# dataexplorations2026/cough_detector

Measured on AMD Instinct MI355X. Metric: 1s@16kHz clips/sec (featurise+infer), higher is better.
Workload: dtype bf16x3: split-bf16 MFMA (feature image, activations and BN-folded weights as hi+lo bf16 pairs, 3 v_mfma_f32_32x32x16_bf16 per k-step, f32 accumulate, f32 activations in HBM); featuriser f32

## Files before the change

### cough_detector_amd/csrc/common.h

```cpp
#pragma once
#include <hip/hip_runtime.h>

#include <cstdarg>
#include <cstdio>

#include "../../include/cough_amd.h"

namespace cough {

void set_error(const char* fmt, ...);

#define COUGH_DEFINE_LAST_ERROR(entry_point)                                  \
    namespace cough {                                                         \
    namespace {                                                               \
    thread_local char g_last_error[512] = "";                                 \
    }                                                                         \
    void set_error(const char* fmt, ...) {                                    \
        va_list ap;                                                           \
        va_start(ap, fmt);                                                    \
        vsnprintf(g_last_error, sizeof(g_last_error), fmt, ap);               \
        va_end(ap);                                                           \
    }                                                                         \
    }                                                                         \
    extern "C" const char* entry_point(void) { return cough::g_last_error; }

inline bool aligned(const void* p, size_t a) { return (reinterpret_cast<size_t>(p) & (a - 1)) == 0; }

#define COUGH_HIP_CHECK(expr)                                                              \
    do {                                                                                   \
        hipError_t _e = (expr);                                                            \
        if (_e != hipSuccess) {                                                            \
            ::cough::set_error("%s failed: %s (%s:%d)", #expr, hipGetErrorString(_e), __FILE__, __LINE__); \
            return COUGH_EHIP;                                                             \
        }                                                                                  \
    } while (0)

#define COUGH_REQUIRE(cond, code, ...)       \
    do {                                     \
        if (!(cond)) {                       \
            ::cough::set_error(__VA_ARGS__); \
            return (code);                   \
        }                                    \
    } while (0)

template <int CTRL, int ROW_MASK = 0xf>
__device__ __forceinline__ float dpp_mov(float v) {
    return __int_as_float(__builtin_amdgcn_update_dpp(0, __float_as_int(v), CTRL, ROW_MASK, 0xf, false));
}
__device__ __forceinline__ float wave_max(float v) {
    v = fmaxf(v, dpp_mov<0xB1>(v));
    v = fmaxf(v, dpp_mov<0x4E>(v));
    v = fmaxf(v, dpp_mov<0x141>(v));
    v = fmaxf(v, dpp_mov<0x140>(v));
    v = fmaxf(v, __shfl_xor(v, 16, 64));
    v = fmaxf(v, __shfl_xor(v, 32, 64));
    return v;
}
__device__ __forceinline__ float wave_sum(float v) {
    v += dpp_mov<0xB1>(v);
    v += dpp_mov<0x4E>(v);
    v += dpp_mov<0x141>(v);
    v += dpp_mov<0x140>(v);
    v += __shfl_xor(v, 16, 64);
    v += __shfl_xor(v, 32, 64);
    return v;
}

__device__ __forceinline__ float mul_rn(float a, float b) {
    float r;
    asm volatile("v_mul_f32 %0, %1, %2" : "=v"(r) : "v"(a), "v"(b));
    return r;
}

__device__ __forceinline__ void wave_lds_fence() {
    __builtin_amdgcn_fence(__ATOMIC_ACQ_REL, "wavefront");
    __builtin_amdgcn_wave_barrier();
}

}
```

### cough_detector_amd/csrc/featurize.hip

```cpp
#include <cmath>
#include <cstddef>
#include <cstring>
#include <type_traits>
#include <vector>

#include <hip/hip_bf16.h>

#include <cstdlib>

#include "common.h"
#include "fft256.h"
#include "internal.h"

namespace cough {
namespace {

constexpr int NS = 16000, NFFT = 512, HOP = 160, WIN = 400, NFRAMES = 101, NMEL = 64, NMFCC = 13;
constexpr int PADL = NFFT / 2;
constexpr int NBIN = 128;
constexpr int MAXW = 8;
constexpr int THREADS = 256, WAVES = THREADS / 64;
constexpr int FPW = 4;
constexpr int NGROUP = (NFRAMES + FPW - 1) / FPW;
constexpr int XROW = 17;
constexpr int XFRAME = 16 * XROW;
constexpr int NMF = NMFCC * NFRAMES;
constexpr int FIRST_PLAIN = 2, LAST_PLAIN = 98;

struct FeatTables {
    float win[NFFT];
    float2 tw256[16][16];
    float2 tw512[NBIN];
    int mel_start[NMEL];
    float mel_w[NMEL][MAXW];
    float dct_t[NMFCC + 1][NMEL];
};

constexpr size_t LDS_XCH = size_t(WAVES) * FPW * XFRAME * 4;
constexpr size_t LDS_MEL = size_t(NMEL) * NFRAMES * 4;
constexpr size_t LDS_RED = 16 * 4;
constexpr size_t LDS_TW = size_t(16) * XROW * 8;
constexpr size_t LDS_TOTAL = LDS_XCH + LDS_MEL + LDS_RED + LDS_TW;
static_assert(LDS_TOTAL * 3 <= 160 * 1024, "three workgroups per CU");
static_assert(LDS_XCH >= size_t(2) * NMF * 4, "MFCC / delta buffers alias the transpose scratch");

__device__ __forceinline__ float block_max(float v, float* red, int tid) {
    v = wave_max(v);
    __syncthreads();
    if ((tid & 63) == 0) red[tid >> 6] = v;
    __syncthreads();
    float r = red[0];
#pragma unroll
    for (int w = 1; w < WAVES; ++w) r = fmaxf(r, red[w]);
    return r;
}
__device__ __forceinline__ float block_sum(float v, float* red, int tid) {
    v = wave_sum(v);
    __syncthreads();
    if ((tid & 63) == 0) red[tid >> 6] = v;
    __syncthreads();
    float r = red[0];
#pragma unroll
    for (int w = 1; w < WAVES; ++w) r += red[w];
    return r;
}

#ifdef COUGH_K1_STAMPS
__device__ unsigned long long* g_stamp_buf = nullptr;
#define K1_STAMP(slot)                                                                      \
    do {                                                                                    \
        if (g_stamp_buf && threadIdx.x == 0)                                                \
            g_stamp_buf[(size_t)blockIdx.x * 8 + (slot)] = __builtin_amdgcn_s_memtime();    \
    } while (0)
#else
#define K1_STAMP(slot) do { } while (0)
#endif

#ifdef COUGH_K1_MARKERS
#define K1_MARK(text)                             \
    do {                                          \
        __builtin_amdgcn_sched_barrier(0);        \
        asm volatile("; K1MARK " text);           \
        __builtin_amdgcn_sched_barrier(0);        \
    } while (0)
#else
#define K1_MARK(text) do { } while (0)
#endif

using f32x16 = __attribute__((ext_vector_type(16))) float;
using bf16x8 = __attribute__((ext_vector_type(8))) __bf16;
__device__ __forceinline__ uint16_t f2bf(float f) {
    __hip_bfloat16 b = __float2bfloat16(f);
    return *reinterpret_cast<uint16_t*>(&b);
}
constexpr int ST_P1H = 22, ST_P1W = 25, ST_ROWS = 94;
constexpr int ST_PER = ST_P1H * ST_P1W, ST_TILES = (ST_PER + 7) / 8;
constexpr int ST_PITCH_NARROW = 106, ST_PITCH_WIDE = 112;
constexpr int st_pitch(bool full) { return full ? ST_PITCH_NARROW : ST_PITCH_WIDE; }
constexpr size_t st_img(bool full) { return size_t(ST_ROWS) * st_pitch(full) * 2; }
static_assert((2 * (ST_PITCH_WIDE / 2)) % 32 == 16 && ST_PITCH_WIDE % 2 == 0, "wide pitch: dy moves a fragment 16 banks on");
static_assert(st_img(false) <= LDS_MEL, "the bf16 feature image aliases the dB buffer");
constexpr size_t LDS_WG3_MAX = 53760;
constexpr size_t st_x3_off(bool full) { return full ? LDS_TOTAL - 2 * st_img(true) : (size_t(NMF) * 4 + 15) & ~size_t(15); }
constexpr size_t LDS_X3_WIDE = st_x3_off(false) + 2 * st_img(false);
static_assert(st_x3_off(false) % 16 == 0 && st_x3_off(true) % 16 == 0 && st_img(false) % 4 == 0 && st_img(true) % 4 == 0 &&
              st_x3_off(true) >= size_t(NMF) * 4, "hi / lo images vs the MFCC buffer");
static_assert(LDS_X3_WIDE >= LDS_TOTAL && LDS_X3_WIDE <= LDS_WG3_MAX, "the widened split-bf16 stem keeps three workgroups per CU");
constexpr size_t shipped_lds_bytes(int stem) { return stem == 2 ? LDS_X3_WIDE : LDS_TOTAL; }

struct FullBank {
    int n_mels, n_mfcc, n_taps;
    int maxw[2];
    int n_frames, n_samples, hop;
    int cph, cph_pad, cw;
    const int *lo, *hi, *off;
    const float* w;
    const float* dct;
};
constexpr size_t full_mel_bytes(int n_mels, int n_frames = NFRAMES) { return (size_t(n_mels) * n_frames * 4 + 15) & ~size_t(15); }
constexpr int FX_ROW = FPW * 16 + 1, FX_WAVE = 16 * FX_ROW, FX_PROW = 260;
static_assert(FPW * FX_PROW <= FX_WAVE && FX_PROW >= NFFT / 2 + 2 && FX_PROW % 2 == 0, "four power rows replace the transposes");
constexpr size_t LDS_XCH_FULL = size_t(WAVES) * FX_WAVE * 4;
constexpr int FULL_MAX_MFCC = int(LDS_XCH_FULL / (size_t(2) * NFRAMES * 4));
constexpr size_t full_lds_bytes(int n_mels, int n_taps, int n_frames = NFRAMES) {
    return LDS_XCH_FULL + full_mel_bytes(n_mels, n_frames) + LDS_RED + LDS_TW + ((size_t(n_taps) * 4 + 15) & ~size_t(15));
}

#ifndef COUGH_GEO_WG_PER_CU
#define COUGH_GEO_WG_PER_CU 2
#endif
template <bool PRE_EMPH, int STEM, bool FULL = false, bool TALL = false, bool PCS = false, bool GEO = false>
__global__ __launch_bounds__(THREADS, GEO ? COUGH_GEO_WG_PER_CU : 3) void featurize_kernel(
    const float* __restrict__ wav, long long wav_stride, float* __restrict__ out, int nfeat,
    const FeatTables* __restrict__ tb, int normalize, float pre_coef, int delta_delta , int pcen, StemFuse stem, FullBank fbk,
    const float* __restrict__ full_dct ,
    float* __restrict__ peak_out ) {
    extern __shared__ __attribute__((aligned(16))) char smem[];
    static_assert(!GEO || (FULL && STEM == 0 && !TALL && !PCS), "run-time geometry: full-band instantiations without a stem");
    constexpr int ST_PITCH = st_pitch(FULL);
    constexpr size_t ST_X3_OFF = st_x3_off(FULL);
    static_assert(FULL || shipped_lds_bytes(STEM) <= LDS_WG3_MAX, "a shipped instantiation keeps three workgroups per CU");
    const int NF = GEO ? fbk.n_frames : NFRAMES, NGR = GEO ? (fbk.n_frames + FPW - 1) / FPW : NGROUP;
    const int NSMP = GEO ? fbk.n_samples : NS, HP = GEO ? fbk.hop : HOP;
    constexpr int N1A = GEO ? 0 : 1, N1B = GEO ? 16 : 15;
    const int nmel = FULL ? fbk.n_mels : NMEL, nmfcc = FULL ? fbk.n_mfcc : NMFCC, nmf = nmfcc * NF;
    const size_t lds_mel = FULL ? full_mel_bytes(nmel, NF) : LDS_MEL;
    constexpr size_t lds_xch = FULL ? LDS_XCH_FULL : LDS_XCH;
    float* xs = reinterpret_cast<float*>(smem);
    float* melbuf = reinterpret_cast<float*>(smem + lds_xch);
    float* red = reinterpret_cast<float*>(smem + lds_xch + lds_mel);
    float2* twl = reinterpret_cast<float2*>(smem + lds_xch + lds_mel + LDS_RED);
    float* c_w = reinterpret_cast<float*>(smem + lds_xch + lds_mel + LDS_RED + LDS_TW);

    const int tid = threadIdx.x, lane = tid & 63, wave = tid >> 6;
    const long long clip = blockIdx.x;
    const float* x = wav + clip * wav_stride;
    float* o = out + clip * (long long)nfeat * NF;
    const bool wr = out != nullptr;

    K1_STAMP(0);
    K1_STAMP(1);
    K1_MARK("PHASE prologue (window taps, twiddle table, mel taps to registers)");

    const int j = lane & 15, fsub = lane >> 4;
    twl[(tid >> 4) * XROW + (tid & 15)] = tb->tw256[tid >> 4][tid & 15];
    int b_lo[2] = {0, 0}, b_w[2] = {0, 0}, b_band[2] = {0, 0};
    const float* b_taps[2] = {c_w, c_w};
    int fpl1 = FPW;
    if constexpr (FULL) {
        for (int i = tid; i < fbk.n_taps; i += THREADS) c_w[i] = fbk.w[i];
        const int r = nmel - 64;
        fpl1 = r > 32 ? 4 : r > 16 ? 2 : 1;
#pragma unroll
        for (int ps = 0; ps < 2; ++ps) {
            const int mb = ps == 0 ? lane : 64 + (fpl1 == 4 ? lane : fpl1 == 2 ? (lane & 31) : (lane & 15));
            if (mb < nmel) {
                b_band[ps] = mb;
                b_lo[ps] = fbk.lo[mb];
                b_w[ps] = fbk.hi[mb] - b_lo[ps];
                b_taps[ps] = c_w + fbk.off[mb];
            } else {
                b_band[ps] = -1;
            }
        }
    }
    __syncthreads();
    const float2* tw_row = twl + j * XROW;
    const float2 tw_j = tb->tw512[j];
    float mw[MAXW];
#pragma unroll
    for (int q = 0; q < MAXW; ++q) mw[q] = tb->mel_w[lane][q];
    const int mstart = tb->mel_start[lane];

    float* myx = xs + (wave * FPW + fsub) * XFRAME;
    float* myw = xs + wave * FX_WAVE;
    float* fxw = myw + 16 * fsub + j;
    const float* fxr = myw + FX_ROW * j + 16 * fsub;
    float* prow = myw + FX_PROW * fsub;
    float run_max = -INFINITY;
    float peak = 0.f;
    float chk = 0.f;
    auto geo_plain = [&](int g) {
        return HP * (FPW * g) - PADL >= 0 && FPW * g + FPW - 1 < NF && HP * (FPW * g + FPW - 1) - PADL + NFFT <= NSMP;
    };
    [[maybe_unused]] float raw_left = 0.f;
    auto load_group = [&](int g, float2 (&raw)[16]) {
        const int t_raw = FPW * g + fsub;
        const int t = t_raw < NF ? t_raw : NF - 1;
        const int s0 = HP * t - PADL + 2 * j;
        if constexpr (GEO) {
            if (geo_plain(g)) {
#pragma unroll
                for (int n1 = 0; n1 < 16; ++n1) raw[n1] = make_float2(x[s0 + 32 * n1], x[s0 + 32 * n1 + 1]);
                if constexpr (PRE_EMPH) raw_left = s0 - 2 * j > 0 ? x[s0 - 2 * j - 1] : 0.f;
            } else {
#pragma unroll
                for (int n1 = 0; n1 < 16; ++n1) {
                    int i0 = s0 + 32 * n1, i1 = i0 + 1;
                    i0 = i0 < 0 ? -i0 : (i0 >= NSMP ? 2 * (NSMP - 1) - i0 : i0);
                    i1 = i1 < 0 ? -i1 : (i1 >= NSMP ? 2 * (NSMP - 1) - i1 : i1);
                    raw[n1] = make_float2(x[i0], x[i1]);
                }
            }
        } else
        if (FPW * g >= FIRST_PLAIN && FPW * g + FPW - 1 <= LAST_PLAIN) {
            K1_MARK("WEIGHT 0.885 (23 of 26 groups: frames inside the clip)");
#pragma unroll
            for (int n1 = 1; n1 < 15; ++n1) raw[n1] = *reinterpret_cast<const float2*>(x + s0 + 32 * n1);
            K1_MARK("ENDWEIGHT");
        } else {
            K1_MARK("WEIGHT 0.115 (3 of 26 groups: reflected edge frames)");
#pragma unroll
            for (int n1 = 1; n1 < 15; ++n1) {
                int i0 = s0 + 32 * n1, i1 = i0 + 1;
                i0 = i0 < 0 ? -i0 : (i0 >= NS ? 2 * (NS - 1) - i0 : i0);
                i1 = i1 < 0 ? -i1 : (i1 >= NS ? 2 * (NS - 1) - i1 : i1);
                raw[n1] = make_float2(x[i0], x[i1]);
            }
            K1_MARK("ENDWEIGHT");
        }
    };
    float2 raw[16];
    float peak_m = 0.f;
    auto p1_pass = [&](const float ws1, const float ws2) {
        float w_re[16], w_im[16];
        const int jw = 2 * j;
#pragma unroll
        for (int n1 = N1A; n1 < N1B; ++n1) {
            w_re[n1] = tb->win[32 * n1 + jw] * ws1 * ws2;
            w_im[n1] = tb->win[32 * n1 + jw + 1] * ws1 * ws2;
        }
        load_group(wave, raw);

        K1_MARK("LOOP 6.5 P1 four-frame groups per wave");
        for (int g = wave; g < NGR; g += WAVES) {
            K1_MARK("PHASE P1 peak + window multiply + next group's loads");
            const int t_raw = FPW * g + fsub;
            const int t = t_raw < NF ? t_raw : NF - 1;
            const int s0 = HP * t - PADL + 2 * j;
            float2 a[16];
            if constexpr (!GEO) {
                a[0] = make_float2(0.f, 0.f);
                a[15] = make_float2(0.f, 0.f);
            }
            if constexpr (!PRE_EMPH) {
#pragma unroll
                for (int n1 = N1A; n1 < N1B; ++n1) {
                    peak = fmaxf(peak, fmaxf(fabsf(raw[n1].x), fabsf(raw[n1].y)));
                    a[n1] = make_float2(raw[n1].x * w_re[n1], raw[n1].y * w_im[n1]);
                }
            }
            if constexpr (PRE_EMPH) {
                if (GEO ? geo_plain(g) : (FPW * g >= FIRST_PLAIN && FPW * g + FPW - 1 <= LAST_PLAIN)) {
                    float carry = GEO ? raw_left : 0.f;
#pragma unroll
                    for (int n1 = N1A; n1 < N1B; ++n1) {
                        const float rot = dpp_mov<0x121>(raw[n1].y);
                        const float left = j == 0 ? carry : rot;
                        carry = rot;
                        const float x0 = raw[n1].x, x1 = raw[n1].y;
                        peak = fmaxf(peak, fmaxf(fabsf(x0), fabsf(x1)));
                        a[n1] = make_float2(__fsub_rn(x0, mul_rn(pre_coef, left)) * w_re[n1],
                                            __fsub_rn(x1, mul_rn(pre_coef, x0)) * w_im[n1]);
                    }
                } else {
#pragma unroll
                    for (int n1 = N1A; n1 < N1B; ++n1) {
                        int i0 = s0 + 32 * n1, i1 = i0 + 1;
                        i0 = i0 < 0 ? -i0 : (i0 >= NSMP ? 2 * (NSMP - 1) - i0 : i0);
                        i1 = i1 < 0 ? -i1 : (i1 >= NSMP ? 2 * (NSMP - 1) - i1 : i1);
                        const float p0 = i0 > 0 ? mul_rn(pre_coef, x[i0 - 1]) : 0.f;
                        const float p1 = i1 > 0 ? mul_rn(pre_coef, x[i1 - 1]) : 0.f;
                        const float x0 = raw[n1].x, x1 = raw[n1].y;
                        peak = fmaxf(peak, fmaxf(fabsf(x0), fabsf(x1)));
                        a[n1] = make_float2(__fsub_rn(x0, p0) * w_re[n1], __fsub_rn(x1, p1) * w_im[n1]);
                    }
                }
            }
            if (g + WAVES < NGR) load_group(g + WAVES, raw);
            K1_MARK("PHASE P1 radix-16 #1");
            dft16(a);
            K1_MARK("PHASE P1 twiddle (LDS table) complex multiply");
#pragma unroll
            for (int k1 = 1; k1 < 16; ++k1) a[k1] = cmul(a[k1], tw_row[k1]);
            K1_MARK("PHASE P1 16x16 transpose through LDS");
            float2 z[16];
#pragma unroll
            for (int k1 = 0; k1 < 16; ++k1) (FULL ? fxw[k1 * FX_ROW] : myx[k1 * XROW + j]) = a[k1].x;
            wave_lds_fence();
#pragma unroll
            for (int n2 = 0; n2 < 16; ++n2) z[n2].x = FULL ? fxr[n2] : myx[j * XROW + n2];
            wave_lds_fence();
#pragma unroll
            for (int k1 = 0; k1 < 16; ++k1) (FULL ? fxw[k1 * FX_ROW] : myx[k1 * XROW + j]) = a[k1].y;
            wave_lds_fence();
#pragma unroll
            for (int n2 = 0; n2 < 16; ++n2) z[n2].y = FULL ? fxr[n2] : myx[j * XROW + n2];
            K1_MARK("PHASE P1 radix-16 #2");
            dft16(z);
            K1_MARK("PHASE P1 real-input split + |X|^2 -> LDS");

            float2 rv[8];
#pragma unroll
            for (int r = 0; r < 8; ++r) {
                rv[r].x = dpp_mov<0x121>(dpp_mov<0x140>(z[8 + r].x));
                rv[r].y = dpp_mov<0x121>(dpp_mov<0x140>(z[8 + r].y));
            }
            wave_lds_fence();
            if constexpr (!FULL) {
#pragma unroll
                for (int k2 = 0; k2 < 8; ++k2) {
                    const float2 zk = z[k2];
                    const float2 zp0 = (k2 == 0) ? z[0] : rv[8 - k2];
                    const float2 zp = (j == 0) ? zp0 : rv[7 - k2];
                    const float ex = zk.x + zp.x, ey = zk.y - zp.y;
                    const float ox = zk.y + zp.y, oy = zp.x - zk.x;
                    const float qx = W32C[k2] * ox - W32S[k2] * oy, qy = W32C[k2] * oy + W32S[k2] * ox;
                    const float xr = ex + tw_j.x * qx - tw_j.y * qy;
                    const float xi = ey + tw_j.x * qy + tw_j.y * qx;
                    myx[j + 16 * k2] = xr * xr + xi * xi;
                }
                wave_lds_fence();
                K1_MARK("PHASE P1 sparse mel + log2 -> LDS");
#pragma unroll
                for (int f = 0; f < FPW; ++f) {
                    const float* p = xs + (wave * FPW + f) * XFRAME + mstart;
                    float acc = 0.f;
#pragma unroll
                    for (int q = 0; q < MAXW; ++q) acc += mw[q] * p[q];
                    const int tf = FPW * g + f;
                    if (tf < NF) {
                        const float db = 3.01029995663981195f * __log2f(acc);
                        melbuf[lane * NF + tf] = db;
                        run_max = fmaxf(run_max, db);
                        chk = fmaf(acc, 0.f, chk);
                    }
                }
            } else {
#pragma unroll
                for (int k2 = 0; k2 < 8; ++k2) {
                    const float2 zk = z[k2];
                    const float2 zp0 = (k2 == 0) ? z[0] : rv[8 - k2];
                    const float2 zp = (j == 0) ? zp0 : rv[7 - k2];
                    const float ex = zk.x + zp.x, ey = zk.y - zp.y;
                    const float ox = zk.y + zp.y, oy = zp.x - zk.x;
                    const float qx = W32C[k2] * ox - W32S[k2] * oy, qy = W32C[k2] * oy + W32S[k2] * ox;
                    const float px = tw_j.x * qx - tw_j.y * qy, py = tw_j.x * qy + tw_j.y * qx;
                    const float ar = ex + px, ai = ey + py, br = ex - px, bi = ey - py;
                    prow[j + 16 * k2] = ar * ar + ai * ai;
                    prow[NFFT / 2 - (j + 16 * k2)] = br * br + bi * bi;
                }
                if (j == 0) prow[NFFT / 4] = 4.0f * (z[8].x * z[8].x + z[8].y * z[8].y);
                wave_lds_fence();
                K1_MARK("PHASE P1 CSR mel + log2 -> LDS");
                auto mel_pass = [&](auto fpl_tag, int ps) {
                    constexpr int FPL = decltype(fpl_tag)::value;
                    const int f0 = FPL == 4 ? 0 : FPL == 2 ? 2 * (lane >> 5) : (lane >> 4);
                    const int mb = b_band[ps], wdt = mb >= 0 ? b_w[ps] : 0;
                    const float* wm = b_taps[ps];
                    const float* p0 = myw + f0 * FX_PROW + b_lo[ps];
                    float acc[FPL];
#pragma unroll
                    for (int f = 0; f < FPL; ++f) acc[f] = 0.f;
                    const int wmax = fbk.maxw[ps];
                    const int lastp = wdt > 2 ? wdt - 2 : 0;
                    for (int k0 = 0; k0 < wmax; k0 += 4) {
                        float2 w[2], pw[2][FPL];
#pragma unroll
                        for (int u = 0; u < 2; ++u) {
                            const int k = k0 + 2 * u, kk = k < lastp ? k : lastp;
                            w[u] = *reinterpret_cast<const float2*>(wm + kk);
#pragma unroll
                            for (int f = 0; f < FPL; ++f) pw[u][f] = *reinterpret_cast<const float2*>(p0 + f * FX_PROW + kk);
                            if (k >= wdt) w[u] = make_float2(0.f, 0.f);
                        }
#pragma unroll
                        for (int u = 0; u < 2; ++u)
#pragma unroll
                            for (int f = 0; f < FPL; ++f) acc[f] = fmaf(w[u].y, pw[u][f].y, fmaf(w[u].x, pw[u][f].x, acc[f]));
                    }
#pragma unroll
                    for (int f = 0; f < FPL; ++f) {
                        const int tf = FPW * g + f0 + f;
                        if (mb >= 0 && tf < NF) {
                            const float db = 3.01029995663981195f * __log2f(acc[f]);
                            melbuf[mb * NF + tf] = db;
                            run_max = fmaxf(run_max, db);
                            chk = fmaf(acc[f], 0.f, chk);
                        }
                    }
                };
                mel_pass(std::integral_constant<int, 4>{}, 0);
                if (nmel > 64) {
                    if (fpl1 == 4) mel_pass(std::integral_constant<int, 4>{}, 1);
                    else if (fpl1 == 2) mel_pass(std::integral_constant<int, 2>{}, 1);
                    else mel_pass(std::integral_constant<int, 1>{}, 1);
                }
            }
            wave_lds_fence();
        }
    };
    p1_pass(1.f, 1.f);

    K1_MARK("ENDLOOP");
    K1_MARK("PHASE P2 block max / peak, shift and floor");
    K1_STAMP(2);
    if (normalize) {
        peak_m = block_max(peak, red, tid);
        if (peak_out != nullptr && tid == 0) peak_out[clip] = peak_m;
        const int pe = (__float_as_int(peak_m) >> 23) & 0xff;
        if ((pe < 127 - 50 || pe > 127 + 50) && peak_m != 0.f && pe != 255) {
            const int e = pe ? pe - 127 : -127 - __builtin_clz(__float_as_int(peak_m) << 9);
            const int k = (e > 0 ? 40 : -40) - e;
            const float ws1 = __int_as_float((127 + k / 2) << 23);
            const float ws2 = __int_as_float((127 + k - k / 2) << 23);
            peak_m = peak_m * ws1 * ws2;
            run_max = -INFINITY;
            chk = 0.f;
            __syncthreads();
            p1_pass(ws1, ws2);
        }
    }
    if (chk != chk) run_max = INFINITY;
    const float raw_max = block_max(run_max, red, tid);
    if (raw_max == INFINITY) {
        const float nanv = __builtin_nanf("");
        const int rows = nmel + (delta_delta == 2 ? 0 : (delta_delta == 1 ? 3 : 2) * nmfcc);
        if (wr)
            for (int i = tid; i < rows * NF; i += THREADS) o[i] = nanv;
        if constexpr (STEM != 0)
            if (tid == 0) stem.nanflag[clip] = 1;
        return;
    }
    if constexpr (STEM != 0)
        if (tid == 0) stem.nanflag[clip] = 0;
    float shift = 0.f;
    if (normalize && peak_m > 0.f) shift = 20.0f * log10f(peak_m);
    const float floor_db = fmaxf(raw_max - shift, -100.0f) - 80.0f;
    K1_STAMP(3);
    bool wr_mel = wr;
    [[maybe_unused]] float pcv[PCS ? 26 : 1];
    K1_MARK("SKIP PCEN branch (off in the shipped configuration)");
    if (GEO && pcen) {
        const int mt = tid >> 2, quarter = (NF + 3) >> 2;
        const int q0 = (tid & 3) * quarter;
        float lmin = INFINITY, lmax = -INFINITY;
        auto pcen_chunk = [&](int mm, int c, int qe, float (&pv)[26]) {
            const int t0 = q0 + 26 * c;
            float p[36], s2[35];
#pragma unroll
            for (int k = 0; k < 36; ++k) {
                const int u = t0 - 5 + k;
                p[k] = (u >= 0 && u < NF) ? exp2f((melbuf[mm * NF + u] - shift) * 0.33219280948873623f) : 0.f;
            }
#pragma unroll
            for (int k = 0; k < 35; ++k) s2[k] = p[k] + p[k + 1];
#pragma unroll
            for (int k = 0; k < 26; ++k) {
                const float sm = ((s2[k] + s2[k + 2]) + (s2[k + 4] + s2[k + 6])) + s2[k + 8];
                const float gain = __builtin_amdgcn_exp2f(-0.98f * __builtin_amdgcn_logf(1e-6f + sm * 0.1f));
                pv[k] = __builtin_amdgcn_sqrtf(fmaf(p[k + 5], gain, 2.0f)) - 1.41421356237309515f;
                if (t0 + k < qe) {
                    lmin = fminf(lmin, pv[k]);
                    lmax = fmaxf(lmax, pv[k]);
                }
            }
        };
        const int m = mt < nmel ? mt : 0;
        const int q1 = mt >= nmel ? q0 : q0 + quarter < NF ? q0 + quarter : NF;
        float pv[2][26];
        pcen_chunk(m, 0, q1, pv[0]);
        if (quarter > 26) pcen_chunk(m, 1, q1, pv[1]);
        const int m2 = mt + 64 < nmel ? mt + 64 : 0;
        const int q2 = mt + 64 >= nmel ? q0 : q0 + quarter < NF ? q0 + quarter : NF;
        if (nmel > 64) {
#pragma unroll 1
            for (int c = 0; c < 2; ++c) {
                if (c == 0 || quarter > 26) {
                    float pw[26];
                    pcen_chunk(m2, c, q2, pw);
#pragma unroll
                    for (int k = 0; k < 26; ++k)
                        if (q0 + 26 * c + k < q2) o[m2 * NF + q0 + 26 * c + k] = pw[k];
                }
            }
        }
        const float mn = -block_max(-lmin, red, tid), mx = block_max(lmax, red, tid);
        const float rng = 1.0f / (mx - mn + 1e-8f);
#pragma unroll
        for (int c = 0; c < 2; ++c)
#pragma unroll
            for (int k = 0; k < 26; ++k)
                if (q0 + 26 * c + k < q1) o[m * NF + q0 + 26 * c + k] = (pv[c][k] - mn) * rng;
        for (int t = q0; t < q2; ++t) o[m2 * NF + t] = (o[m2 * NF + t] - mn) * rng;
        wr_mel = false;
    } else
    if (pcen) {
        const int m = tid >> 2, t0 = (tid & 3) * 26, t1 = t0 + 26 < NF ? t0 + 26 : NF;
        float p[36], pv[26];
#pragma unroll
        for (int k = 0; k < 36; ++k) {
            const int u = t0 - 5 + k;
            p[k] = (u >= 0 && u < NF) ? exp2f((melbuf[m * NF + u] - shift) * 0.33219280948873623f) : 0.f;
        }
        float lmin = INFINITY, lmax = -INFINITY;
        float s2[35];
#pragma unroll
        for (int k = 0; k < 35; ++k) s2[k] = p[k] + p[k + 1];
#pragma unroll
        for (int k = 0; k < 26; ++k) {
            const float sm = ((s2[k] + s2[k + 2]) + (s2[k + 4] + s2[k + 6])) + s2[k + 8];
            const float gain = __builtin_amdgcn_exp2f(-0.98f * __builtin_amdgcn_logf(1e-6f + sm * 0.1f));
            pv[k] = __builtin_amdgcn_sqrtf(fmaf(p[k + 5], gain, 2.0f)) - 1.41421356237309515f;
            if (t0 + k < t1) { lmin = fminf(lmin, pv[k]); lmax = fmaxf(lmax, pv[k]); }
        }
        const float mn = -block_max(-lmin, red, tid), mx = block_max(lmax, red, tid);
        const float rng = 1.0f / (mx - mn + 1e-8f);
        if (wr) {
#pragma unroll
            for (int k = 0; k < 26; ++k)
                if (t0 + k < t1) o[m * NF + t0 + k] = (pv[k] - mn) * rng;
        }
        if constexpr (PCS) {
#pragma unroll
            for (int k = 0; k < 26; ++k) pcv[k] = (pv[k] - mn) * rng;
        }
        wr_mel = false;
    }
    K1_MARK("ENDSKIP");
    K1_MARK("PHASE P2 floor + mel rows store");
    if constexpr (GEO) {
        for (int i = tid; i < nmel * NF; i += THREADS) {
            const float d = fmaxf(fmaxf(melbuf[i] - shift, -100.0f), floor_db);
            melbuf[i] = d;
            if (wr_mel) o[i] = fminf(fmaxf((d + 80.0f) * 0.0125f, 0.f), 1.f);
        }
    } else
    for (int i2 = tid; i2 < nmel * NFRAMES / 2; i2 += THREADS) {
        float2 d = reinterpret_cast<float2*>(melbuf)[i2];
        d.x = fmaxf(fmaxf(d.x - shift, -100.0f), floor_db);
        d.y = fmaxf(fmaxf(d.y - shift, -100.0f), floor_db);
        reinterpret_cast<float2*>(melbuf)[i2] = d;
        float2 v;
        v.x = fminf(fmaxf((d.x + 80.0f) * 0.0125f, 0.f), 1.f);
        v.y = fminf(fmaxf((d.y + 80.0f) * 0.0125f, 0.f), 1.f);
        if (wr_mel) reinterpret_cast<float2*>(o)[i2] = v;
    }
    __syncthreads();
    K1_STAMP(4);
    if (delta_delta == 2) return;
    K1_MARK("PHASE P2 DCT 13x64");
    float* mf = xs;
    float* dl = GEO ? melbuf : mf + nmf;
    const int tt0 = tid & 127;
    const int chalf = __builtin_amdgcn_readfirstlane(tid >> 7);
    if constexpr (FULL) {
        const int cph = fbk.cph, nch = chalf ? nmfcc - cph : cph, cbase = chalf * cph;
        auto dct_chunks = [&](auto cw_tag) {
            constexpr int CW = decltype(cw_tag)::value;
            for (int tt = tt0; tt < (GEO ? ((NF + 127) & ~127) : 128); tt += 128)
            for (int cq = 0; cq < nch; cq += CW) {
                float acc[CW];
#pragma unroll
                for (int cc = 0; cc < CW; ++cc) acc[cc] = 0.f;
                if (tt < NF) {
                    const float* drow = full_dct + (size_t(chalf) * fbk.cph_pad + cq) / CW * size_t(nmel) * 8;
#pragma unroll 8
                    for (int m = 0; m < nmel; ++m) {
                        const float v = melbuf[m * NF + tt];
#pragma unroll
                        for (int cc = 0; cc < CW; ++cc) acc[cc] = fmaf(drow[m * 8 + cc], v, acc[cc]);
                    }
#pragma unroll
// ... 62 lines not shown
    };
    if constexpr (TALL) {
        static_assert(!TALL || STEM == 2, "the 103-row stem: split-bf16 operands");
        constexpr int TL_P1H = 26, TL_HALF = 13, TL_PER = TL_HALF * ST_P1W, TL_ROWS = 58, TL_PLANE = TL_ROWS * ST_PITCH;
        constexpr size_t TL_IMG_OFF = (size_t(2) * NMF * 4 + 15) & ~size_t(15), TL_STASH_OFF = TL_IMG_OFF + size_t(2) * TL_PLANE * 2;
        constexpr int TL_KEEP0 = 2 * 2 * TL_HALF - 3;
        static_assert(TL_STASH_OFF % 16 == 0 && TL_STASH_OFF + size_t(NMEL - TL_KEEP0) * NFRAMES * 4 <= LDS_TOTAL, "103-row stem LDS");
        static_assert(2 * (2 * (TL_HALF - 1) + 1) + 1 + 6 < TL_ROWS && TL_P1H == 2 * TL_HALF, "partial image rows");
        constexpr int NDV = (NMEL * NFRAMES / 2 + THREADS - 1) / THREADS;
        float2 dv[NDV];
#pragma unroll
        for (int it = 0; it < NDV; ++it) {
            const int i2 = tid + it * THREADS;
            dv[it] = i2 < NMEL * NFRAMES / 2 ? reinterpret_cast<const float2*>(melbuf)[i2] : make_float2(0.f, 0.f);
        }
        float* o_mfcc = o + NMEL * NFRAMES;
        float* o_delta = o_mfcc + NMF;
        for (int item = tid; item < NMF; item += THREADS) {
            const int c = item / NFRAMES, t = item - c * NFRAMES;
            const float* row = mf + c * NFRAMES;
            const float d = (row[t < NFRAMES - 1 ? t + 1 : t] - row[t > 0 ? t - 1 : 0]) / 2.0f;
            if (wr) {
                o_mfcc[item] = row[t];
                o_delta[item] = d;
            }
            dl[item] = d;
        }
        __syncthreads();
        auto ddelta = [&](int c, int t) {
            const float* row = dl + c * NFRAMES;
            return (row[t < NFRAMES - 1 ? t + 1 : t] - row[t > 0 ? t - 1 : 0]) / 2.0f;
        };
        if (wr) {
            float* o_dd = o_delta + NMF;
            for (int item = tid; item < NMF; item += THREADS) o_dd[item] = ddelta(item / NFRAMES, item % NFRAMES);
        }
        uint16_t* timg = reinterpret_cast<uint16_t*>(smem + TL_IMG_OFF);
        float* stash = reinterpret_cast<float*>(smem + TL_STASH_OFF);
        auto tput = [&](int idx, float v) {
            const uint16_t hi = f2bf(v);
            timg[idx] = hi;
            timg[TL_PLANE + idx] = f2bf(v - __uint_as_float(uint32_t(hi) << 16));
        };
        auto zero_image = [&]() {
            for (int i = tid; i < 2 * TL_PLANE / 8; i += THREADS) reinterpret_cast<uint4*>(timg)[i] = make_uint4(0, 0, 0, 0);
            for (int i = (2 * TL_PLANE / 8) * 8 + tid; i < 2 * TL_PLANE; i += THREADS) timg[i] = 0;
            __syncthreads();
        };
        zero_image();
        if constexpr (PCS) {
            const int m = tid >> 2, t0 = (tid & 3) * 26;
#pragma unroll
            for (int k = 0; k < 26; ++k) {
                if (t0 + k < NFRAMES) {
                    if (m + 3 < TL_ROWS - 1) tput((m + 3) * ST_PITCH + t0 + k + 3, pcv[k]);
                    if (m >= TL_KEEP0) stash[(m - TL_KEEP0) * NFRAMES + t0 + k] = pcv[k];
                }
            }
        } else {
            {
#pragma unroll
                for (int it = 0; it < NDV; ++it) {
                    const int e = 2 * (tid + it * THREADS);
                    if (e < NMEL * NFRAMES) {
                        const int m0 = e / NFRAMES, t0 = e - m0 * NFRAMES;
                        const int m1 = t0 + 1 < NFRAMES ? m0 : m0 + 1, t1 = t0 + 1 < NFRAMES ? t0 + 1 : 0;
                        const float v0 = fminf(fmaxf((dv[it].x + 80.0f) * 0.0125f, 0.f), 1.f);
                        const float v1 = fminf(fmaxf((dv[it].y + 80.0f) * 0.0125f, 0.f), 1.f);
                        if (m0 + 3 < TL_ROWS - 1) tput((m0 + 3) * ST_PITCH + t0 + 3, v0);
                        if (m1 + 3 < TL_ROWS - 1) tput((m1 + 3) * ST_PITCH + t1 + 3, v1);
                        if (m0 >= TL_KEEP0) stash[(m0 - TL_KEEP0) * NFRAMES + t0] = v0;
                        if (m1 >= TL_KEEP0) stash[(m1 - TL_KEEP0) * NFRAMES + t1] = v1;
                    }
                }
            }
        }
        const int sr = lane & 31, sh = lane >> 5;
        bf16x8 bw[2][4];
#pragma unroll
        for (int pl = 0; pl < 2; ++pl)
#pragma unroll
            for (int st = 0; st < 4; ++st)
                bw[pl][st] = *reinterpret_cast<const bf16x8*>(stem.wfrag + pl * 2048 + ((st * 2 + sh) * 32 + sr) * 8);
        const float bn = stem.bias[sr];
        const int q = sr >> 2, dy = (sr >> 1) & 1, dx = sr & 1;
        float* oa = reinterpret_cast<float*>(stem.a1) + clip * (long long)(TL_P1H * ST_P1W) * 32;
#pragma unroll 1
        for (int half = 0; half < 2; ++half) {
            if (half == 1) {
                zero_image();
                for (int i = tid; i < (NMEL - TL_KEEP0) * NFRAMES; i += THREADS) {
                    const int m = i / NFRAMES, t = i - m * NFRAMES;
                    tput(m * ST_PITCH + t + 3, stash[i]);
                }
                for (int item = tid; item < NMF; item += THREADS) {
                    const int c = item / NFRAMES, t = item - c * NFRAMES;
                    tput((NMEL - TL_KEEP0 + c) * ST_PITCH + t + 3, mf[item]);
                    tput((NMEL - TL_KEEP0 + NMFCC + c) * ST_PITCH + t + 3, dl[item]);
                    tput((NMEL - TL_KEEP0 + 2 * NMFCC + c) * ST_PITCH + t + 3, ddelta(c, t));
                }
            }
            __syncthreads();
            auto tl_base = [&](int tile) -> const uint32_t* {
                int P = tile * 8 + q;
                if (P >= TL_PER) P = TL_PER - 1;
                const int ph = P / ST_P1W, pw = P - ph * ST_P1W;
                return reinterpret_cast<const uint32_t*>(timg + (2 * (2 * ph + dy) + sh) * ST_PITCH + 2 * (2 * pw + dx));
            };
            auto tl_load = [&](const uint32_t* base, bf16x8 (&fa)[2][4]) {
#pragma unroll
                for (int pl = 0; pl < 2; ++pl)
#pragma unroll
                    for (int st = 0; st < 4; ++st) {
                        const uint32_t* pp = base + pl * (TL_PLANE / 2) + st * ST_PITCH;
                        union { uint32_t u[4]; bf16x8 v; } tv;
                        tv.u[0] = pp[0]; tv.u[1] = pp[1]; tv.u[2] = pp[2]; tv.u[3] = pp[3];
                        fa[pl][st] = tv.v;
                    }
            };
            auto tl_mma = [&](const bf16x8 (&fa)[2][4], f32x16& c) {
#pragma unroll
                for (int st = 0; st < 4; ++st) {
                    c = __builtin_amdgcn_mfma_f32_32x32x16_bf16(fa[0][st], bw[0][st], c, 0, 0, 0);
                    c = __builtin_amdgcn_mfma_f32_32x32x16_bf16(fa[1][st], bw[0][st], c, 0, 0, 0);
                    c = __builtin_amdgcn_mfma_f32_32x32x16_bf16(fa[0][st], bw[1][st], c, 0, 0, 0);
                }
            };
            auto tl_store = [&](int tile, const f32x16& acc2) {
#pragma unroll
                for (int g = 0; g < 4; ++g) {
                    const int Po = tile * 8 + 2 * g + sh;
                    float v = fmaxf(fmaxf(acc2[4 * g], acc2[4 * g + 1]), fmaxf(acc2[4 * g + 2], acc2[4 * g + 3])) + bn;
                    v = fmaxf(v, 0.f);
                    if (Po < TL_PER) oa[(half * TL_PER + Po) * 32 + sr] = v;
                }
            };
            constexpr int TL_TILES = (TL_PER + 7) / 8;
            for (int ta = wave; ta < TL_TILES; ta += 2 * WAVES) {
                const int tb = ta + WAVES;
                const bool two = tb < TL_TILES;
                bf16x8 fa[2][4], fb[2][4];
                tl_load(tl_base(ta), fa);
                tl_load(tl_base(two ? tb : ta), fb);
                f32x16 ca = {0}, cb = {0};
                tl_mma(fa, ca);
                tl_mma(fb, cb);
                tl_store(ta, ca);
                if (two) tl_store(tb, cb);
            }
            __syncthreads();
        }
        return;
    }
    if constexpr (STEM != 0) {
        float2 dv[(NMEL * NFRAMES / 2 + THREADS - 1) / THREADS];
#pragma unroll
        for (int it = 0; it < (NMEL * NFRAMES / 2 + THREADS - 1) / THREADS; ++it) {
            const int i2 = tid + it * THREADS;
            dv[it] = i2 < NMEL * NFRAMES / 2 ? reinterpret_cast<const float2*>(melbuf)[i2] : make_float2(0.f, 0.f);
        }
        __syncthreads();
        constexpr int NIMG = STEM == 2 ? 2 : 1;
        for (int i = tid; i < NIMG * ST_ROWS * ST_PITCH / 8; i += THREADS) reinterpret_cast<uint4*>(img)[i] = make_uint4(0, 0, 0, 0);
        for (int i = (NIMG * ST_ROWS * ST_PITCH / 8) * 8 + tid; i < NIMG * ST_ROWS * ST_PITCH; i += THREADS) img[i] = 0;
        __syncthreads();
        if constexpr (PCS) {
            const int m = tid >> 2, t0 = (tid & 3) * 26;
#pragma unroll
            for (int k = 0; k < 26; ++k)
                if (t0 + k < NFRAMES) put((m + 3) * ST_PITCH + t0 + k + 3, pcv[k]);
        } else {
#pragma unroll
            for (int it = 0; it < (NMEL * NFRAMES / 2 + THREADS - 1) / THREADS; ++it) {
                const int e = 2 * (tid + it * THREADS);
                if (e < NMEL * NFRAMES) {
                    const int m0 = e / NFRAMES, t0 = e - m0 * NFRAMES;
                    const int m1 = t0 + 1 < NFRAMES ? m0 : m0 + 1, t1 = t0 + 1 < NFRAMES ? t0 + 1 : 0;
                    put((m0 + 3) * ST_PITCH + t0 + 3, fminf(fmaxf((dv[it].x + 80.0f) * 0.0125f, 0.f), 1.f));
                    put((m1 + 3) * ST_PITCH + t1 + 3, fminf(fmaxf((dv[it].y + 80.0f) * 0.0125f, 0.f), 1.f));
                }
            }
        }
    }
    float* o_mfcc = o + nmel * NF;
    float* o_delta = o_mfcc + nmf;
    for (int item = tid; item < nmf; item += THREADS) {
        const int c = item / NF, t = item - c * NF;
        const float* row = mf + c * NF;
        const float d = (row[t < NF - 1 ? t + 1 : t] - row[t > 0 ? t - 1 : 0]) / 2.0f;
        if (wr) {
            o_mfcc[item] = row[t];
            o_delta[item] = d;
        }
        if (delta_delta == 1) dl[item] = d;
        if constexpr (STEM != 0) {
            put((NMEL + c + 3) * ST_PITCH + t + 3, row[t]);
            put((NMEL + NMFCC + c + 3) * ST_PITCH + t + 3, d);
        }
    }
    K1_STAMP(6);
    if (delta_delta == 1 && wr) {
        __syncthreads();
        float* o_dd = o_delta + nmf;
        for (int item = tid; item < nmf; item += THREADS) {
            const int c = item / NF, t = item - c * NF;
            const float* row = dl + c * NF;
            o_dd[item] = (row[t < NF - 1 ? t + 1 : t] - row[t > 0 ? t - 1 : 0]) / 2.0f;
        }
    }
    if constexpr (STEM != 0) {
        __syncthreads();
        K1_MARK("PHASE K2 stem MFMA + pool + store");
        constexpr int NP = STEM == 2 ? 2 : 1;
        const int sr = lane & 31, sh = lane >> 5;
        bf16x8 bw[NP][4];
#pragma unroll
        for (int pl = 0; pl < NP; ++pl)
#pragma unroll
            for (int st = 0; st < 4; ++st)
                bw[pl][st] = *reinterpret_cast<const bf16x8*>(stem.wfrag + pl * 2048 + ((st * 2 + sh) * 32 + sr) * 8);
        const float bn = stem.bias[sr];
        const int q = sr >> 2, dy = (sr >> 1) & 1, dx = sr & 1;
        using out_t = std::conditional_t<STEM == 2, float, uint16_t>;
        out_t* oa = reinterpret_cast<out_t*>(stem.a1) + clip * (long long)ST_PER * 32;
        constexpr uint32_t IMG_OFF = STEM == 2 ? uint32_t(ST_X3_OFF) : uint32_t(lds_xch);
        auto frag_base = [&](int tile) -> uint32_t {
            int P = tile * 8 + q;
            if (P >= ST_PER) P = ST_PER - 1;
            const int ph = P / ST_P1W, pw = P - ph * ST_P1W;
            return IMG_OFF + 2 * uint32_t((2 * (2 * ph + dy) + sh) * ST_PITCH + 2 * (2 * pw + dx));
        };
        static_assert(4 * ST_PITCH + 12 <= 1020, "both k-steps of a pair within ds_read2_b32's reach");
        auto load_frags = [&](uint32_t base, bf16x8 (&a)[NP][4]) {
#pragma unroll
            for (int pl = 0; pl < NP; ++pl)
#pragma unroll
                for (int sp = 0; sp < 2; ++sp) {
                    using lds_u32 = const __attribute__((address_space(3))) uint32_t;
                    lds_u32* p = (lds_u32*)(smem + (base + pl * (ST_ROWS * ST_PITCH * 2) + sp * (8 * ST_PITCH)));
                    asm("" : "+v"(p));
#pragma unroll
                    for (int s2 = 0; s2 < 2; ++s2) {
                        union { uint32_t u[4]; bf16x8 v; } t;
                        t.u[0] = p[s2 * ST_PITCH]; t.u[1] = p[s2 * ST_PITCH + 1];
                        t.u[2] = p[s2 * ST_PITCH + 2]; t.u[3] = p[s2 * ST_PITCH + 3];
                        a[pl][2 * sp + s2] = t.v;
                    }
                }
        };
        auto mma = [&](const bf16x8 (&a)[NP][4], f32x16& c) {
#pragma unroll
            for (int st = 0; st < 4; ++st) {
                c = __builtin_amdgcn_mfma_f32_32x32x16_bf16(a[0][st], bw[0][st], c, 0, 0, 0);
                if constexpr (STEM == 2) {
                    c = __builtin_amdgcn_mfma_f32_32x32x16_bf16(a[1][st], bw[0][st], c, 0, 0, 0);
                    c = __builtin_amdgcn_mfma_f32_32x32x16_bf16(a[0][st], bw[1][st], c, 0, 0, 0);
                }
            }
        };
        auto epilogue = [&](int tile, const f32x16& acc2, bool guard) {
#pragma unroll
            for (int g = 0; g < 4; ++g) {
                const int Po = tile * 8 + 2 * g + sh;
                float v = fmaxf(fmaxf(acc2[4 * g], acc2[4 * g + 1]), fmaxf(acc2[4 * g + 2], acc2[4 * g + 3])) + bn;
                v = fmaxf(v, 0.f);
                if (!guard || Po < ST_PER) {
                    if constexpr (STEM == 2) oa[Po * 32 + sr] = v;
                    else oa[Po * 32 + sr] = f2bf(v);
                }
            }
        };
        static_assert(ST_TILES == 17 * WAVES + 1, "stem tile split");
        for (int it = 0; it < 16; it += 2) {
            const int ta = wave + WAVES * it, tbb = ta + WAVES;
            bf16x8 fa[NP][4], fb[NP][4];
            load_frags(frag_base(ta), fa);
            load_frags(frag_base(tbb), fb);
            f32x16 ca = {0}, cb = {0};
            mma(fa, ca);
            mma(fb, cb);
            epilogue(ta, ca, false);
            epilogue(tbb, cb, false);
        }
        {
            const int ta = wave + WAVES * 16;
            const bool last = wave == 0;
            bf16x8 fa[NP][4], fb[NP][4];
            load_frags(frag_base(ta), fa);
            load_frags(frag_base(last ? ST_TILES - 1 : ta), fb);
            f32x16 ca = {0}, cb = {0};
            mma(fa, ca);
            mma(fb, cb);
            epilogue(ta, ca, false);
            if (last) epilogue(ST_TILES - 1, cb, true);
        }
        K1_STAMP(7);
    }
}

}
}

struct cough_featurizer {
    cough_feat_config cfg;
    cough::FeatTables* d_tables;
    float* d_win_full;
    int nfeat;
    int nbase;
    cough::ContrastCfg contrast;
    int n_cus;
    int path;
    char* d_full;
    cough::FullBank full;
    cough::GenFeat* gen;
};

namespace cough {
namespace {
bool geo_basic(const cough_feat_config& c) {
    return c.n_fft == NFFT && c.win_length >= 1 && c.win_length <= NFFT && c.hop_length >= 1 && c.n_mels >= 2 && c.n_mels <= 128 &&
           (!c.use_mfcc || (c.n_mfcc >= 1 && c.n_mfcc <= c.n_mels));
}
bool geo_fits(const cough_feat_config& c, int n_taps, int n) {
    if (n <= NFFT / 2) return false;
    const long long T = n / c.hop_length + 1;
    const bool covered = c.hop_length <= NFFT / 2 || (c.hop_length <= NFFT && (T - 1) * c.hop_length + NFFT / 2 >= n);
    return covered && T <= 1024 && (!c.use_pcen || T <= 208) && (!c.use_mfcc || size_t(c.n_mfcc) * T * 4 <= LDS_XCH_FULL) &&
           full_lds_bytes(c.n_mels, n_taps, int(T)) <= 80 * 1024;
}

using K1Fn = decltype(&featurize_kernel<false, 0>);
struct K1Entry {
    bool pe;
    int stem;
    bool full, tall, pcs, geo;
    K1Fn fn;
};
#define K1(PE, STEM, FULL, TALL, PCS, GEO) {PE, STEM, FULL, TALL, PCS, GEO, featurize_kernel<PE, STEM, FULL, TALL, PCS, GEO>}
#define K1_X3(FULL, PCS) K1(false, 2, FULL, false, PCS, false), K1(false, 2, FULL, true, PCS, false), \
                        K1(true, 2, FULL, false, PCS, false), K1(true, 2, FULL, true, PCS, false)
const K1Entry K1_TABLE[] = {
    K1(false, 0, true, false, false, false), K1(true, 0, true, false, false, false),
    K1_X3(true, false), K1_X3(true, true),
    K1(false, 0, true, false, false, true), K1(true, 0, true, false, false, true),
    K1_X3(false, false), K1_X3(false, true),
    K1(false, 1, false, false, false, false),
    K1(true, 0, false, false, false, false), K1(false, 0, false, false, false, false),
};
#undef K1_X3
#undef K1
// ... 314 lines not shown
```

Before: 6.587 million.

## Hoist peak tracking, pair-pack stem image writes, tighten DPP moves

Several independent changes land together. The per-frame peak tracking is moved out of the window-multiply loop, using v_max3 with absolute-value modifiers and skipping pairs that overlap the previous frame. The next group's loads are moved after the first radix-16 DFT, with asm barriers that fix the schedule. The stem feature-image fill is rewritten to write bf16 pixel pairs as 32-bit words: only the border is zeroed instead of the whole image, and MFCC and delta rows are computed directly from register windows. The f32 MFCC/delta output loop is now skipped when not needed. DPP moves switch to mov_dpp with bound_ctrl, guarded by a static_assert. These changes trade extra code complexity and index-boundary risk for fewer LDS stores, fewer ALU ops and fewer barriers in the featuriser.

```diff
diff --git a/cough_detector_amd/csrc/common.h b/cough_detector_amd/csrc/common.h
--- a/cough_detector_amd/csrc/common.h
+++ b/cough_detector_amd/csrc/common.h
@@ -43,9 +43,15 @@
         }                                    \
     } while (0)
 
-template <int CTRL, int ROW_MASK = 0xf>
+constexpr bool dpp_full_row_permutation(int ctrl) {
+    return ctrl == 0xB1 || ctrl == 0x4E
+        || ctrl == 0x141 || ctrl == 0x140
+        || ctrl == 0x121;
+}
+template <int CTRL>
 __device__ __forceinline__ float dpp_mov(float v) {
-    return __int_as_float(__builtin_amdgcn_update_dpp(0, __float_as_int(v), CTRL, ROW_MASK, 0xf, false));
+    static_assert(dpp_full_row_permutation(CTRL), "dpp_mov: the control must permute the whole row (old is undefined)");
+    return __int_as_float(__builtin_amdgcn_mov_dpp(__float_as_int(v), CTRL, 0xf, 0xf, true));
 }
 __device__ __forceinline__ float wave_max(float v) {
     v = fmaxf(v, dpp_mov<0xB1>(v));
diff --git a/cough_detector_amd/csrc/featurize.hip b/cough_detector_amd/csrc/featurize.hip
--- a/cough_detector_amd/csrc/featurize.hip
+++ b/cough_detector_amd/csrc/featurize.hip
@@ -86,6 +86,14 @@
 #else
 #define K1_MARK(text) do { } while (0)
 #endif
+
+__device__ __forceinline__ float max3_abs(float m, float a, float b) {
+    float r;
+    asm("v_max3_f32 %0, %1, |%2|, |%3|" : "=v"(r) : "v"(m), "v"(a), "v"(b));
+    return r;
+}
+constexpr int PEAK_N1 = 9;
+static_assert(32 * PEAK_N1 <= 32 * 15 - HOP, "the pairs from PEAK_N1 on join the previous frame's");
 
 using f32x16 = __attribute__((ext_vector_type(16))) float;
 using bf16x8 = __attribute__((ext_vector_type(8))) __bf16;
@@ -251,10 +259,16 @@
             w_im[n1] = tb->win[32 * n1 + jw + 1] * ws1 * ws2;
         }
         load_group(wave, raw);
+        if constexpr (!GEO) {
+            if (wave == 0) {
+#pragma unroll
+                for (int n1 = N1A; n1 < PEAK_N1; ++n1) peak = max3_abs(peak, raw[n1].x, raw[n1].y);
+            }
+        }
 
         K1_MARK("LOOP 6.5 P1 four-frame groups per wave");
         for (int g = wave; g < NGR; g += WAVES) {
-            K1_MARK("PHASE P1 peak + window multiply + next group's loads");
+            K1_MARK("PHASE P1 peak + window multiply");
             const int t_raw = FPW * g + fsub;
             const int t = t_raw < NF ? t_raw : NF - 1;
             const int s0 = HP * t - PADL + 2 * j;
@@ -263,12 +277,16 @@
                 a[0] = make_float2(0.f, 0.f);
                 a[15] = make_float2(0.f, 0.f);
             }
+            if constexpr (GEO) {
+#pragma unroll
+                for (int n1 = N1A; n1 < N1B; ++n1) peak = fmaxf(peak, fmaxf(fabsf(raw[n1].x), fabsf(raw[n1].y)));
+            } else {
+#pragma unroll
+                for (int n1 = PEAK_N1; n1 < N1B; ++n1) peak = max3_abs(peak, raw[n1].x, raw[n1].y);
+            }
             if constexpr (!PRE_EMPH) {
 #pragma unroll
-                for (int n1 = N1A; n1 < N1B; ++n1) {
-                    peak = fmaxf(peak, fmaxf(fabsf(raw[n1].x), fabsf(raw[n1].y)));
-                    a[n1] = make_float2(raw[n1].x * w_re[n1], raw[n1].y * w_im[n1]);
-                }
+                for (int n1 = N1A; n1 < N1B; ++n1) a[n1] = make_float2(raw[n1].x * w_re[n1], raw[n1].y * w_im[n1]);
             }
             if constexpr (PRE_EMPH) {
                 if (GEO ? geo_plain(g) : (FPW * g >= FIRST_PLAIN && FPW * g + FPW - 1 <= LAST_PLAIN)) {
@@ -279,7 +297,6 @@
                         const float left = j == 0 ? carry : rot;
                         carry = rot;
                         const float x0 = raw[n1].x, x1 = raw[n1].y;
-                        peak = fmaxf(peak, fmaxf(fabsf(x0), fabsf(x1)));
                         a[n1] = make_float2(__fsub_rn(x0, mul_rn(pre_coef, left)) * w_re[n1],
                                             __fsub_rn(x1, mul_rn(pre_coef, x0)) * w_im[n1]);
                     }
@@ -292,14 +309,16 @@
                         const float p0 = i0 > 0 ? mul_rn(pre_coef, x[i0 - 1]) : 0.f;
                         const float p1 = i1 > 0 ? mul_rn(pre_coef, x[i1 - 1]) : 0.f;
                         const float x0 = raw[n1].x, x1 = raw[n1].y;
-                        peak = fmaxf(peak, fmaxf(fabsf(x0), fabsf(x1)));
                         a[n1] = make_float2(__fsub_rn(x0, p0) * w_re[n1], __fsub_rn(x1, p1) * w_im[n1]);
                     }
                 }
             }
+            K1_MARK("PHASE P1 radix-16 #1 + next group's loads");
+            dft16(a);
+            asm volatile("" : "+v"(peak));
+#pragma unroll
+            for (int k1 = 0; k1 < 16; ++k1) asm volatile("" : "+v"(a[k1].x), "+v"(a[k1].y));
             if (g + WAVES < NGR) load_group(g + WAVES, raw);
-            K1_MARK("PHASE P1 radix-16 #1");
-            dft16(a);
             K1_MARK("PHASE P1 twiddle (LDS table) complex multiply");
 #pragma unroll
             for (int k1 = 1; k1 < 16; ++k1) a[k1] = cmul(a[k1], tw_row[k1]);
@@ -438,7 +457,9 @@
             run_max = -INFINITY;
             chk = 0.f;
             __syncthreads();
+            K1_MARK("SKIP rescaled second P1 pass (a peak outside 2^-50 .. 2^50: never audio)");
             p1_pass(ws1, ws2);
+            K1_MARK("ENDSKIP");
         }
     }
     if (chk != chk) run_max = INFINITY;
@@ -807,50 +828,104 @@
         }
         return;
     }
-    if constexpr (STEM != 0) {
-        float2 dv[(NMEL * NFRAMES / 2 + THREADS - 1) / THREADS];
-#pragma unroll
-        for (int it = 0; it < (NMEL * NFRAMES / 2 + THREADS - 1) / THREADS; ++it) {
-            const int i2 = tid + it * THREADS;
-            dv[it] = i2 < NMEL * NFRAMES / 2 ? reinterpret_cast<const float2*>(melbuf)[i2] : make_float2(0.f, 0.f);
-        }
+    if constexpr (STEM != 0 && PCS) {
         __syncthreads();
         constexpr int NIMG = STEM == 2 ? 2 : 1;
         for (int i = tid; i < NIMG * ST_ROWS * ST_PITCH / 8; i += THREADS) reinterpret_cast<uint4*>(img)[i] = make_uint4(0, 0, 0, 0);
         for (int i = (NIMG * ST_ROWS * ST_PITCH / 8) * 8 + tid; i < NIMG * ST_ROWS * ST_PITCH; i += THREADS) img[i] = 0;
         __syncthreads();
-        if constexpr (PCS) {
-            const int m = tid >> 2, t0 = (tid & 3) * 26;
-#pragma unroll
-            for (int k = 0; k < 26; ++k)
-                if (t0 + k < NFRAMES) put((m + 3) * ST_PITCH + t0 + k + 3, pcv[k]);
-        } else {
-#pragma unroll
-            for (int it = 0; it < (NMEL * NFRAMES / 2 + THREADS - 1) / THREADS; ++it) {
-                const int e = 2 * (tid + it * THREADS);
-                if (e < NMEL * NFRAMES) {
-                    const int m0 = e / NFRAMES, t0 = e - m0 * NFRAMES;
-                    const int m1 = t0 + 1 < NFRAMES ? m0 : m0 + 1, t1 = t0 + 1 < NFRAMES ? t0 + 1 : 0;
-                    put((m0 + 3) * ST_PITCH + t0 + 3, fminf(fmaxf((dv[it].x + 80.0f) * 0.0125f, 0.f), 1.f));
-                    put((m1 + 3) * ST_PITCH + t1 + 3, fminf(fmaxf((dv[it].y + 80.0f) * 0.0125f, 0.f), 1.f));
+        const int m = tid >> 2, t0 = (tid & 3) * 26;
+#pragma unroll
+        for (int k = 0; k < 26; ++k)
+            if (t0 + k < NFRAMES) put((m + 3) * ST_PITCH + t0 + k + 3, pcv[k]);
+    }
+    constexpr int ST_P2 = ST_PITCH / 2, ST_PLANE2 = ST_ROWS * ST_P2, ST_NPAIR = (NFRAMES + 3) / 2;
+    static_assert(ST_PITCH % 2 == 0 && 2 * ST_NPAIR + 2 <= ST_PITCH && NFRAMES % 2 == 1, "pixel pairs: frame 100 ends pair 50");
+    uint32_t* img2 = reinterpret_cast<uint32_t*>(img);
+    [[maybe_unused]] auto put2 = [&](int d , float v0, float v1) {
+        using f32x2 = __attribute__((ext_vector_type(2))) float;
+        using bf16x2 = __attribute__((ext_vector_type(2))) __bf16;
+        const f32x2 v = {v0, v1};
+        const uint32_t hi = __builtin_bit_cast(uint32_t, __builtin_convertvector(v, bf16x2));
+        img2[d] = hi;
+        if constexpr (STEM == 2) {
+            const f32x2 lo = {v0 - __uint_as_float(hi << 16), v1 - __uint_as_float(hi & 0xffff0000u)};
+            img2[ST_PLANE2 + d] = __builtin_bit_cast(uint32_t, __builtin_convertvector(lo, bf16x2));
+        }
+    };
+    [[maybe_unused]] auto zero2 = [&](int d) {
+        img2[d] = 0;
+        if constexpr (STEM == 2) img2[ST_PLANE2 + d] = 0;
+    };
+    if constexpr (STEM != 0 && !PCS) {
+        static_assert(NMEL * 4 == THREADS && 4 * 13 == ST_NPAIR && 4 * ST_P2 <= THREADS, "mel rows of the image: 13 pairs per thread");
+        const int m = tid >> 2, q = tid & 3;
+        const float* src = melbuf + m * NFRAMES + 26 * q - 1;
+        float dv[26];
+#pragma unroll
+        for (int i = 0; i < 26; ++i) {
+            const bool border = (i == 0 && q == 0) || (i >= 24 && q == 3);
+            dv[i] = src[(i == 0 || i >= 24) && border ? 1 : i];
+        }
+        __syncthreads();
+        if (tid < 3 * ST_P2) zero2(tid);
+        else if (tid < 4 * ST_P2) zero2((ST_ROWS - 1) * ST_P2 + tid - 3 * ST_P2);
+        const int row2 = (m + 3) * ST_P2;
+        if (q == 0) zero2(row2);
+        if (q == 3)
+            for (int c = ST_NPAIR + 1; c < ST_P2; ++c) zero2(row2 + c);
+#pragma unroll
+        for (int k = 0; k < 13; ++k) {
+            float v0 = fminf(fmaxf((dv[2 * k] + 80.0f) * 0.0125f, 0.f), 1.f);
+            float v1 = fminf(fmaxf((dv[2 * k + 1] + 80.0f) * 0.0125f, 0.f), 1.f);
+            if (k == 0) v0 = q == 0 ? 0.f : v0;
+            if (k == 12) {
+                v0 = q == 3 ? 0.f : v0;
+                v1 = q == 3 ? 0.f : v1;
+            }
+            put2(row2 + 1 + 13 * q + k, v0, v1);
+        }
+    }
+    if constexpr (STEM != 0) {
+        static_assert(16 * 4 >= ST_P2 - 1 && NMFCC * 16 <= THREADS, "MFCC / delta rows of the image: 4 pairs per thread");
+        const int c = tid >> 4, s = tid & 15;
+        if (c < NMFCC) {
+            const float* row = mf + c * NFRAMES;
+            float xv[10];
+#pragma unroll
+            for (int i = 0; i < 10; ++i) {
+                const int t = 8 * s - 2 + i;
+                xv[i] = row[t < 0 ? 0 : t > NFRAMES - 1 ? NFRAMES - 1 : t];
+            }
+            const int r_mfcc = (NMEL + c + 3) * ST_P2, r_delta = (NMEL + NMFCC + c + 3) * ST_P2;
+            if (s == 0) {
+                zero2(r_mfcc);
+                zero2(r_delta);
+            }
+#pragma unroll
+            for (int k = 0; k < 4; ++k) {
+                const int p = 4 * s + k, t0 = 2 * p - 1;
+                if (p < ST_P2 - 1) {
+                    const bool live0 = t0 >= 0 && t0 < NFRAMES, live1 = t0 + 1 < NFRAMES;
+                    put2(r_mfcc + 1 + p, live0 ? xv[2 * k + 1] : 0.f, live1 ? xv[2 * k + 2] : 0.f);
+                    put2(r_delta + 1 + p, live0 ? (xv[2 * k + 2] - xv[2 * k]) / 2.0f : 0.f,
+                         live1 ? (xv[2 * k + 3] - xv[2 * k + 1]) / 2.0f : 0.f);
                 }
             }
         }
     }
     float* o_mfcc = o + nmel * NF;
     float* o_delta = o_mfcc + nmf;
-    for (int item = tid; item < nmf; item += THREADS) {
-        const int c = item / NF, t = item - c * NF;
-        const float* row = mf + c * NF;
-        const float d = (row[t < NF - 1 ? t + 1 : t] - row[t > 0 ? t - 1 : 0]) / 2.0f;
-        if (wr) {
-            o_mfcc[item] = row[t];
-            o_delta[item] = d;
-        }
-        if (delta_delta == 1) dl[item] = d;
-        if constexpr (STEM != 0) {
-            put((NMEL + c + 3) * ST_PITCH + t + 3, row[t]);
-            put((NMEL + NMFCC + c + 3) * ST_PITCH + t + 3, d);
+    if (wr || delta_delta == 1) {
+        for (int item = tid; item < nmf; item += THREADS) {
+            const int c = item / NF, t = item - c * NF;
+            const float* row = mf + c * NF;
+            const float d = (row[t < NF - 1 ? t + 1 : t] - row[t > 0 ? t - 1 : 0]) / 2.0f;
+            if (wr) {
+                o_mfcc[item] = row[t];
+                o_delta[item] = d;
+            }
+            if (delta_delta == 1) dl[item] = d;
         }
     }
     K1_STAMP(6);
```

After: 6.768 million (median of 6 runs). +2.7%, better.
